# monahand1023/imageclust

Measured on AMD Instinct MI355X. Metric: images/sec (embed+Ward), higher is better.
Workload: dtype bf16; 1 GPU; the metric's size (configs[2]'s N=100000) on 1 GPU: 100000 synthetic 224x224x3 images (structured, seed 20250217; 100000 on this rank), ResNet50-v1 bf16 batch=256 -> 2048-d pooled E -> Ward min=5 max=50 (merge loop on GPU0) -> cluster ids on host; n_images_total=100000, embed_dim=2048, weights=synthetic seed 1, device=AMD Radeon Graphics (gfx950:sramecc+:xnack-)

## Files before the change

### imageclust_amd/_lib.py

```python
import ctypes as C
import os

import numpy as np

_HERE = os.path.dirname(os.path.abspath(__file__))
SO_PATH = os.environ.get("ICL_SO_PATH") or os.path.join(_HERE, "libimageclust_hip.so")

ICL_OK = 0
ICL_ERR_ARG, ICL_ERR_CONSTRAINT, ICL_ERR_HIP, ICL_ERR_NOMODEL, ICL_ERR_IO, ICL_ERR_UNSUPPORTED, ICL_ERR_OVERSIZE, ICL_ERR_NOMEM = range(1, 9)
HEAD_POOLED, HEAD_DENSE0 = 2048, 1000
PREC_FP32, PREC_BF16, PREC_BF16X3 = 0, 1, 2
UPDATE_EXACT, UPDATE_LW = 0, 1
SYNTH_NOISE, SYNTH_STRUCTURED = 0, 1
TILES_AUTO, TILES_LOCAL, TILES_DISTRIBUTED = 0, 1, 2
MERGE_GPU0, MERGE_SHARDED = 0, 1
CONV_P8_OFF, CONV_P8_AUTO, CONV_P8_ALL = 0, 1, 2
CONV_SPLIT = 16
ROWS_SINGLE, ROWS_EXACT_BATCH, ROWS_LW_BOUND, ROWS_LW_FAST, ROWS_SINGLE_APART = 0, 1, 2, 3, 4
FILE_FAIL_NEXT_LEADER = 0x100
MANY_MID_AUTO, MANY_MID_OFF, MANY_MID_ON = 0, 1, 2
PNG_HOST, PNG_GPU = 0, 1
ENTROPY_HOST, ENTROPY_GPU = 0, 1
K_CONV, K_DIST_EXACT, K_DIST_MFMA, K_ROWMIN, K_UPDATE, K_EMBED_OTHER, K_CONV64 = range(7)
K_NAMES = ["conv_igemm_kernel<*,128>", "ward_dist_exact_kernel", "dist_mfma_kernel", "row_argmin_*_kernel",
# ... 59 lines not shown
    ("icl_jpeg_encode_rgb", _int, [_vp, _i32, _i32, _i32, _vp, _i64, _pi64]),
    ("icl_jpeg_encode_rgb_dev", _int, [_vp, _vp, _vp, _vp, _vp, _i64, _i32, _vp, _i32, _i64, _vp]),
    ("icl_downsize_image_file", _int, [C.c_char_p, _i64, _i32, _vp, _i64, _pi64, _vp]),
    ("icl_downsize_image_mem", _int, [_vp, _i64, _i64, _i32, _vp, _i64, _pi64, _vp]),
    ("icl_downsize_images", _int, [_vp, _vp, _i64, _i64, _i32, _i32, _vp, _i64, _vp, _vp]),
    ("icl_downsize_images_mem", _int, [_vp, _vp, _vp, _i64, _i64, _i32, _i32, _vp, _i64, _vp, _vp]),
    ("icl_last_downsize_stats", _int, [_vp, _pi64, _pi64, _pi64, _pi64, _pi64, _pi64, _vp]),
    ("icl_set_batch", _int, [_vp, _int]),
    ("icl_set_conv_options", _int, [_vp, _int]),
    ("icl_conv_stats", _int, [_vp, _vp, _vp]),
    ("icl_set_forward_prune", _int, [_vp, _int]),
    ("icl_forward_prune_stats", _int, [_vp, _vp]),
    ("icl_set_forward_prune_fused", _int, [_vp, _int]),
    ("icl_forward_prune_fused_stats", _int, [_vp, _vp]),
    ("icl_set_stem_max_blocks", _int, [_vp, _int]),
    ("icl_bottleneck56_sub", _int, [_vp, _vp, _int, _int, _int] + [_vp] * 9 + [_int, _int, _vp]),
    ("icl_conv1x1_mapped", _int, [_vp, _vp, _int, _int, _int, _int, _vp, _int, _vp, _vp, _vp, _int, _vp]),
    ("icl_conv_split_launches", _int, [_vp, _vp]),
    ("icl_conv2d_fused", _int, [_vp, _int, _vp, _int, _int, _int, _vp, _int, _int, _int, _int, _vp, _vp, _vp, _int, _vp]),
    ("icl_conv2d_dual", _int, [_vp, _int, _vp, _int, _int, _int, _vp, _vp, _int, _int, _vp, _int, _int, _vp, _vp, _int, _vp]),
    ("icl_embed_taps", _int, [_vp, _int, _vp, _int, _int, _vp]),
    ("icl_stem_pool", _int, [_vp, _int, _vp, _int, _vp]),
    ("icl_bottleneck56", _int, [_vp, _vp, _int, _int, _int, _int] + [_vp] * 13),
    ("icl_calc_optimal_clusters", _int, [_i64, _i64, _i64, _pi64]),
    ("icl_ward_distance_matrix", _int, [_vp, _vp, _vp, _i64, _i32, _vp, _i64]),
    ("icl_ward_distance_matrix_dev", _int, [_vp, _vp, _vp, _i64, _i32, _vp, _i64]),
    ("icl_merge_centroid", _int, [_vp, _vp, _i64, _vp, _i64, _i32, _vp]),
    ("icl_update_distance_matrix", _int, [_vp, _vp, _i64, _i64, _vp, _vp, _i32, _i64, _i64, _vp, _i64]),
    ("icl_find_closest", _int, [_vp, _vp, _i64, _i64, _pi64, _pi64]),
    ("icl_find_closest_dev", _int, [_vp, _vp, _i64, _i64, _pi64, _pi64]),
    ("icl_group_create", _int, [_pi32, _i32, C.POINTER(_vp)]),
    ("icl_group_destroy", None, [_vp]),
# ... 494 lines not shown

    def set_conv_options(self, p8_mode=1):
        check(self.h, self.L.icl_set_conv_options(self.h, p8_mode))

    def set_forward_prune(self, on=True):
        check(self.h, self.L.icl_set_forward_prune(self.h, 1 if on else 0))

    def forward_prune_stats(self):
        a = C.c_int64(0)
        check(self.h, self.L.icl_forward_prune_stats(self.h, C.byref(a)))
        return a.value

    def set_forward_prune_fused(self, on=True):
        check(self.h, self.L.icl_set_forward_prune_fused(self.h, 1 if on else 0))

    def set_stem_max_blocks(self, max_blocks=0):
        check(self.h, self.L.icl_set_stem_max_blocks(self.h, int(max_blocks)))

    def forward_prune_fused_stats(self):
        a = C.c_int64(0)
        check(self.h, self.L.icl_forward_prune_fused_stats(self.h, C.byref(a)))
        return a.value

    def embed_u8(self, imgs, head=HEAD_POOLED, prec=PREC_FP32):
        imgs = np.ascontiguousarray(imgs, np.uint8).reshape(-1, IMG_BYTES)
        n = imgs.shape[0]
        out = np.empty((n, head), np.float32)
        check(self.h, self.L.icl_embed_u8(self.h, imgs.ctypes.data, n, head, prec, out.ctypes.data))
        return out

# ... 229 lines not shown
        Cout, _, k, _ = w.shape
        Ho = (H + 2 * pad - k) // stride + 1
        y = np.empty((B, Ho, Ho, Cout), np.float32)
        sc = np.ascontiguousarray(scale, np.float32)
        sh = np.ascontiguousarray(shift, np.float32)
        r = None if residual is None else np.ascontiguousarray(residual, np.float32)
        check(self.h, self.L.icl_conv2d_fused(self.h, prec, x.ctypes.data, B, H, Cin, w.ctypes.data, Cout, k, stride, pad,
                                              sc.ctypes.data, sh.ctypes.data, None if r is None else r.ctypes.data,
                                              1 if relu else 0, y.ctypes.data))
        return y

    def conv1x1_mapped(self, x_nhwc, w, scale, shift, y_full, sub, residual=None, relu=True):
        f = lambda a: np.ascontiguousarray(a, np.float32)
        x, w, sc, sh = f(x_nhwc), f(w), f(scale), f(shift)
        y = np.array(y_full, np.float32, order="C", copy=True)
        B, H, _, Cout = y.shape
        Ho = (H - 1) // int(sub) + 1
        Cin = x.shape[3]
        assert x.shape == (B, Ho, Ho, Cin) and w.shape == (Cout, Cin) and sc.shape == (Cout,) and sh.shape == (Cout,)
        r = None if residual is None else f(residual)
        assert r is None or r.shape == y.shape
        check(self.h, self.L.icl_conv1x1_mapped(self.h, x.ctypes.data, B, H, int(sub), Cin, w.ctypes.data, Cout, sc.ctypes.data, sh.ctypes.data,
                                                None if r is None else r.ctypes.data, 1 if relu else 0, y.ctypes.data))
        return y

    def conv2d_dual(self, x_nhwc, w1, x2_nhwc, w2, stride2, scale, shift, relu=True, prec=PREC_FP32):
        f = lambda a: np.ascontiguousarray(a, np.float32)
        x, x2, w1, w2, sc, sh = f(x_nhwc), f(x2_nhwc), f(w1), f(w2), f(scale), f(shift)
        B, Ho, _, Cin = x.shape
        _, H2, _, Cin2 = x2.shape
        Cout = w1.shape[0]
        assert x2.shape[0] == B and w1.shape == (Cout, Cin) and w2.shape == (Cout, Cin2) and sc.shape == (Cout,) and sh.shape == (Cout,)
        y = np.empty((B, Ho, Ho, Cout), np.float32)
        check(self.h, self.L.icl_conv2d_dual(self.h, prec, x.ctypes.data, B, Ho, Cin, w1.ctypes.data, x2.ctypes.data, H2, Cin2, w2.ctypes.data,
                                             int(stride2), Cout, sc.ctypes.data, sh.ctypes.data, 1 if relu else 0, y.ctypes.data))
        return y

# ... 783 lines not shown
```

### imageclust_amd/csrc/conv_p8.h

```cpp
#pragma once
#include "conv_select.h"
#include "mfma_tile.h"
#include "resnet_fused.h"

template <int MW, int NWV>
struct p8_geom {
    static_assert(MW * NWV == 8 && (NWV == 4 || NWV == 2), "8 waves");
    static constexpr int BM = MW * 128, BN = NWV * 64;
    static constexpr int PX = MW, PW = NWV / 2;
    static constexpr int SX = PX * 8192, SW = PW * 8192;
    static constexpr int O_WA = 0, O_XA = SW, O_WB = SW + SX, O_XB = 2 * SW + SX;
    static constexpr int BUF = 2 * (SW + SX);
    static constexpr int LDS = 2 * BUF;
    static constexpr int INFLIGHT = 2 * PW + PX;
    static_assert(INFLIGHT == 6 && LDS <= 160 * 1024, "counted vmcnt(6); the CU's 160 KiB");
};

template <int NP>
__device__ __forceinline__ void p8_dma(const i32x4_t &srd, const unsigned (&voff)[NP], unsigned soff, unsigned lds0)
{
    unsigned keep;
    if constexpr (NP == 1) {
        asm volatile("s_mov_b32 %0, m0\n\ts_mov_b32 m0, %4\n\ts_nop 4\n\tbuffer_load_dwordx4 %1, %2, %3 offen lds\n\ts_mov_b32 m0, %0"
                     : "=&s"(keep)
// ... 22 lines not shown
__global__ __launch_bounds__(512) void conv_p8_kernel(const conv_args p)
{
    static_assert(!(SPLIT && DUAL), "the split form covers single-operand layers");
    static_assert(!(SPLIT && X3), "the split form is bf16 only");
    typedef p8_geom<MW, NWV> G;
    typedef unsigned u32x2_t __attribute__((ext_vector_type(2)));
    constexpr int PX = G::PX, PW = G::PW;
    __shared__ __attribute__((aligned(1024))) unsigned char smem[G::LDS];
    const int tid = threadIdx.x, lane = tid & 63;
    const int wid = __builtin_amdgcn_readfirstlane(tid >> 6);
    const int wr = wid / NWV, wc = wid % NWV;
    const int grp = wid >> 2;
    const int ntile = p.gx * p.gy;
    const int role = SPLIT ? (int)blockIdx.x / ntile : 0;
    const int tile = xcd_remap((int)blockIdx.x - role * ntile, ntile);
    const int m0 = (tile / p.gy) * G::BM, n0 = (tile % p.gy) * G::BN;
    const i32x4_t xsrd = bn56_srd(p.X, (unsigned)((size_t)p.B * p.H * p.W * p.Cin * 2));
    const i32x4_t wsrd = bn56_srd(p.Wt, (unsigned)((size_t)p.Cout * p.K * 2));
    const i32x4_t x2srd = DUAL ? bn56_srd(p.X2, (unsigned)((size_t)p.B * p.H2 * p.W2 * p.Cin2 * 2)) : xsrd;

    unsigned vx[2][PX], vw[2][PW], vx2[DUAL ? 2 : 1][PX], vmask[PX];
#pragma unroll
    for (int j = 0; j < PW; ++j) {
        const int sr = (j * 8 + wid) * 8 + (lane >> 3);
        const unsigned ls16 = (unsigned)(((lane & 7) ^ ((sr >> 1) & 7)) << 4);
#pragma unroll
        for (int h = 0; h < 2; ++h) {
            const int wrow = n0 + (sr >> 5) * 64 + h * 32 + (sr & 31);
            vw[h][j] = (unsigned)wrow * (unsigned)p.K * 2u + ls16;
        }
    }
// ... 364 lines not shown
```

### imageclust_amd/csrc/conv_select.h

```cpp
#pragma once
#include <cstddef>
#include <cstdint>

#include "prune_map.h"

struct conv_args {
    const void *X;
    const void *Wt;
    void *Y;
    const void *R;
    const float *scale;
    const float *shift;
    const void *zero;
    int B, H, W, Cin, Ho, Wo, Cout, KH, KW, stride, pad, relu;
    int64_t M;
    int K;
    int gx, gy;
    const void *X2;
    int H2, W2, Cin2, stride2;
    void *sk_part;
    int *sk_flag;
    int sk_epoch;
    prune_map omap;
};

#define CONV_PREC_FP32 0
#define CONV_PREC_BF16 1
#define CONV_PREC_BF16X3 2
#define CONV_TILE_M 128
#define CONV_ROW_BYTES 128
#define HALO_MAXP 12
#ifndef P8_AUTO_MIN_NT
// ... 204 lines not shown
    *ngroups = g < 1 ? 1 : g;
}
static inline unsigned fwd_stem_blocks(int64_t units, int per_cu, int ncu, int max_blocks = 0)
{
    const int64_t g = units < (int64_t)per_cu * ncu ? units : (int64_t)per_cu * ncu;
    return (unsigned)(max_blocks > 0 && max_blocks < g ? max_blocks : g);
}

struct fwd_opts {
    conv_opts conv;
    int fuse;
    int prune;
    int stem_per_cu;
    int prune_fused = 1;
    int stem_max_blocks = 0;
};

enum fwd_kind { FWD_STEM2_POOL, FWD_STEM_POOL, FWD_STEM, FWD_MAXPOOL, FWD_BNECK56, FWD_CONV, FWD_AVGPOOL, FWD_FC };
enum { FWD_X = 0, FWD_T1 = 1, FWD_T2 = 2, FWD_DS = 3, FWD_Y = 4, FWD_NONE = -1 };

struct fwd_step {
    int kind;
    int layer;
    bool ds;
    bool pruned;
    int sub;
    conv_args a;
    conv_choice c;
    int x, y, r, x2;
    unsigned blocks, threads;
};
struct fwd_plan {
    std::vector<fwd_step> steps;
    int out = FWD_X;
    int H = 56, C = 64;
    int B = 0;
    int pruned = 0;
    const char *err = nullptr;
    int err_layer = 0;
};

static inline bool plan_pruned_block(const icl_conv_rec &r2, const icl_conv_rec &r3, int s, int B, const conv_opts &o, conv_args *p2, conv_args *p3)
{
    if (s <= 1) return false;
    const int prec = CONV_PREC_BF16;
    const conv_args u2 = conv_plain(nullptr, nullptr, nullptr, nullptr, nullptr, nullptr, nullptr, B, r2.hin, r2.cin, r2.cout, r2.k, r2.stride, r2.pad, 1);
    conv_args u3 = conv_plain(nullptr, nullptr, nullptr, nullptr, nullptr, nullptr, nullptr, B, r3.hin, r3.cin, r3.cout, 1, 1, 0, 1);
    *p2 = conv_plain(nullptr, nullptr, nullptr, nullptr, nullptr, nullptr, nullptr, B, r2.hin, r2.cin, r2.cout, r2.k, s, r2.pad, 1);
    *p3 = conv_plain(nullptr, nullptr, nullptr, nullptr, nullptr, nullptr, nullptr, B, p2->Ho, r3.cin, r3.cout, 1, 1, 0, 1);
    u3.R = p3->R = &u3;
    p3->omap = prune_map_make(s, r3.hout, r3.hout);
    if (u2.K != r2.cin * r2.k * r2.k || u3.K != r3.cin || p2->Ho != p3->omap.Ho) return false;
    const bool same = conv_same_arithmetic(conv_select(prec, u2, o), conv_select(prec, *p2, o)) && conv_same_arithmetic(conv_select(prec, u3, o), conv_select(prec, *p3, o));
    p3->R = nullptr;
    return same;
}

static inline fwd_plan forward_make_plan(const icl_conv_rec *recs, int nconv, int prec, int B, bool dense_head, int tap, const fwd_opts &o)
{
    fwd_plan p;
    p.B = B;
    const bool bf16 = prec == CONV_PREC_BF16, x3 = prec == CONV_PREC_BF16X3;
    const int bk = bf16 ? 64 : 32;
    int x = FWD_X, y = FWD_Y;
    auto add = [&](int kind, int layer, int xi, int yi) -> fwd_step & {
        fwd_step s = {};
        s.kind = kind; s.layer = layer; s.x = xi; s.y = yi; s.r = s.x2 = FWD_NONE;
        p.steps.push_back(s);
        return p.steps.back();
    };
// ... 67 lines not shown
            conv(ci + 1, FWD_T1, FWD_T2, FWD_NONE, c2.hin, c2.stride, nullptr, FWD_NONE);
            if (has_ds) {
                const icl_conv_rec &d = recs[ci + 3];
                if (d.cin % bk || c3.cout % 128) return fail("fused downsample shape not supported", ci + 2);
                conv(ci + 2, FWD_T2, y, FWD_NONE, c3.hin, 1, nullptr, x);
            } else {
                conv(ci + 2, FWD_T2, y, x, c3.hin, 1, nullptr, FWD_NONE);
            }
        }
        std::swap(x, y);
        ci = cn;
    }
    for (const fwd_step &s : p.steps)
        if (s.kind == FWD_CONV && s.c.family == CONV_UNSUPPORTED) return fail(s.c.why, s.layer);
    p.out = x;
    if (tap >= 0) return p;
    fwd_step &ap = add(FWD_AVGPOOL, 0, x, FWD_NONE);
    ap.blocks = (unsigned)conv_ceil_div((int64_t)B * 2048, 256);
    ap.threads = 256;
    if (dense_head) {
        fwd_step &fc = add(FWD_FC, 0, FWD_NONE, FWD_NONE);
        const int64_t want = conv_ceil_div((int64_t)B * 1000, 4);
        fc.blocks = (unsigned)(want < 4096 ? want : 4096);
        fc.threads = 256;
    }
    return p;
}
```

### imageclust_amd/csrc/conv_wr.h

```cpp
#pragma once
#include "conv_select.h"
#include "mfma_tile.h"
#include "prune_map.h"
#include "resnet_fused.h"

template <int NP>
__device__ __forceinline__ void wr_dma_chunk(const i32x4_t &srd, unsigned v0, unsigned v1, unsigned soff, unsigned lds0)
{
    unsigned keep;
    if constexpr (NP == 2)
        asm volatile("s_mov_b32 %0, m0\n\ts_mov_b32 m0, %5\n\ts_nop 4\n\tbuffer_load_dwordx4 %1, %3, %4 offen lds\n\t"
                     "s_mov_b32 m0, %6\n\ts_nop 0\n\tbuffer_load_dwordx4 %2, %3, %4 offen lds\n\ts_mov_b32 m0, %0"
                     : "=&s"(keep)
                     : "v"(v0), "v"(v1), "s"(srd), "s"(soff), "s"(lds0), "s"(lds0 + 4096u)
                     : "memory");
    else
        asm volatile("s_mov_b32 %0, m0\n\ts_mov_b32 m0, %4\n\ts_nop 4\n\tbuffer_load_dwordx4 %1, %2, %3 offen lds\n\ts_mov_b32 m0, %0"
                     : "=&s"(keep)
                     : "v"(v0), "s"(srd), "s"(soff), "s"(lds0)
                     : "memory");
}
template <int KC, int PT>
__device__ __forceinline__ void wr_dma(const i32x4_t &srd, unsigned v0, unsigned v1, unsigned lds0)
{
    static_assert(PT == 64 || PT == 32, "64- or 32-pixel tiles");
#pragma unroll
    for (int c = 0; c < KC; ++c) wr_dma_chunk<PT / 32>(srd, v0, v1, 128u * c, lds0 + (unsigned)(PT * 128) * c);
}

struct wr_args {
    const uint16_t *X;
    const uint16_t *W;
    const uint16_t *R;
    uint16_t *Y;
    const float *scale, *shift;
    int M, N, relu;
    int nslices, nworkers;
    prune_map pm;
};

template <int K, int NS, int MT, bool RES, bool MAP = false>
__global__ __launch_bounds__(256, (K == 256 && MT == 2) ? 3 : 2) void conv_wr_kernel(const wr_args p)
{
    typedef unsigned u32x2_t __attribute__((ext_vector_type(2)));
    typedef unsigned u32x4_t __attribute__((ext_vector_type(4)));
    constexpr int KC = K / 64, KF = K / 32;
    constexpr int CW = NS / 4, NT = CW / 16;
    constexpr int PT = 16 * MT;
    constexpr int ABYTES = KC * PT * 128;
    static_assert(NT % 2 == 0 && NT * KF * 4 <= 128 && (MT == 4 || MT == 2), "pairs of accumulator tiles for the lane swap; <= 128 VGPRs of weights");
    __shared__ __attribute__((aligned(1024))) unsigned char smem[2 * ABYTES];
    const int tid = threadIdx.x, lane = tid & 63;
    const int wid = __builtin_amdgcn_readfirstlane(tid >> 6);
    const int l15 = lane & 15, q = lane >> 4;
    const int xcd = (int)blockIdx.x & 7, rr = (int)blockIdx.x >> 3;
    const int slice = rr % p.nslices, worker = (rr / p.nslices) * 8 + xcd;
    const int n0 = slice * NS + wid * CW;
    const int ntiles = (p.M + PT - 1) / PT;
    if (worker >= ntiles) return;

    u32x4_t wreg[NT][KF];
#pragma unroll
    for (int nt = 0; nt < NT; ++nt)
#pragma unroll
        for (int kf = 0; kf < KF; ++kf) wreg[nt][kf] = *reinterpret_cast<const u32x4_t *>(p.W + (size_t)(n0 + 16 * nt + l15) * K + 32 * kf + 8 * q);
    asm volatile("s_waitcnt vmcnt(0)" ::: "memory");
#pragma unroll
    for (int nt = 0; nt < NT; ++nt)
#pragma unroll
        for (int kf = 0; kf < KF; ++kf) asm volatile("" : "+v"(wreg[nt][kf]));
    const int cbl = (q & 1) * 16 + (q >> 1) * 8;
    float sc[NT / 2][8], sh[NT / 2][8];
#pragma unroll
    for (int i = 0; i < NT / 2; ++i) {
// ... 4 lines not shown
        sh[i][0] = b0.x; sh[i][1] = b0.y; sh[i][2] = b0.z; sh[i][3] = b0.w; sh[i][4] = b1.x; sh[i][5] = b1.y; sh[i][6] = b1.z; sh[i][7] = b1.w;
    }
    const i32x4_t xsrd = bn56_srd(p.X, (unsigned)((size_t)p.M * K * 2));
    const unsigned lds0 = __builtin_amdgcn_readfirstlane(lds_addr_of(smem) + wid * 1024);
    int drow[2];
    unsigned dsw[2];
#pragma unroll
    for (int j = 0; j < 2; ++j) {
        drow[j] = (j * 4 + wid) * 8 + (lane >> 3);
        dsw[j] = (unsigned)(((lane & 7) ^ ((drow[j] >> 1) & 7)) << 4);
    }
    auto stage = [&](int tile, int buf) {
        unsigned v[2];
#pragma unroll
        for (int j = 0; j < 2; ++j) {
            const int m = tile * PT + drow[j];
            v[j] = (tile < ntiles && m < p.M) ? (unsigned)m * (unsigned)(K * 2) + dsw[j] : BN56_OOB;
        }
        wr_dma<KC, PT>(xsrd, v[0], v[1], lds0 + buf * ABYTES);
    };
    const int fsw = (l15 >> 1) & 7;
    unsigned xoff[2];
#pragma unroll
    for (int s = 0; s < 2; ++s) xoff[s] = (unsigned)(l15 * 128 + ((((4 * s + q) ^ fsw) & 7) << 4));

    typedef uint16_t elem;
    const size_t ypix = MAP ? (size_t)(p.M / (p.pm.Ho * p.pm.Wo)) * p.pm.H * p.pm.W : (size_t)p.M;
    const __amdgpu_buffer_rsrc_t rsrd = __builtin_amdgcn_make_buffer_rsrc((void *)(RES ? p.R : p.Y), 0, (int)(ypix * p.N * 2), 0x00020000);
    const __amdgpu_buffer_rsrc_t ysrd = __builtin_amdgcn_make_buffer_rsrc((void *)p.Y, 0, (int)(ypix * p.N * 2), 0x00020000);
    u32x4_t rv[MT][NT / 2];
    auto row_off = [&](int tile, int mt) -> unsigned {
        const int64_t m = (int64_t)tile * PT + mt * 16 + l15;
        if constexpr (MAP) {
            if (!(tile < ntiles && m < p.M)) return BN56_OOB;
            return (unsigned)((prune_map_pixel(p.pm, (unsigned)m) * p.N + n0 + cbl) * 2);
        }
        return (tile < ntiles && m < p.M) ? (unsigned)((m * p.N + n0 + cbl) * 2) : BN56_OOB;
    };
    auto load_res = [&](int tile) {
        if (!RES) return;
#pragma unroll
        for (int mt = 0; mt < MT; ++mt) {
            const unsigned o = row_off(tile, mt);
#pragma unroll
            for (int i = 0; i < NT / 2; ++i) rv[mt][i] = __builtin_amdgcn_raw_buffer_load_b128(rsrd, (int)o, i * 64, 0);
        }
    };
// ... 76 lines not shown
        }
        return;
    }
    if (res) hipLaunchKernelGGL((conv_wr_kernel<K, NS, MT, true>), grid, dim3(256), 0, strm, w);
    else hipLaunchKernelGGL((conv_wr_kernel<K, NS, MT, false>), grid, dim3(256), 0, strm, w);
}
static void launch_conv_wr(icl_ctx *ctx, const conv_args &a, const conv_choice &c)
{
    hipStream_t strm = ctx->cur_stream ? ctx->cur_stream : ctx->stream;
    wr_args w;
    w.X = (const uint16_t *)a.X; w.W = (const uint16_t *)a.Wt; w.R = (const uint16_t *)a.R; w.Y = (uint16_t *)a.Y;
    w.scale = a.scale; w.shift = a.shift; w.M = (int)a.M; w.N = a.Cout; w.relu = a.relu;
    w.pm = a.omap;
    w.nslices = c.slices;
    w.nworkers = c.workers;
    const dim3 grid(c.blocks);
    if (c.wr_k == 128) launch_conv_wr_t<128, 256, 4>(strm, w, grid, c.res);
    else if (c.wr_k == 256 && c.wr_mt == 4) launch_conv_wr_t<256, 128, 4>(strm, w, grid, c.res);
    else if (c.wr_k == 256) launch_conv_wr_t<256, 128, 2>(strm, w, grid, c.res);
    else launch_conv_wr_t<512, 128, 2>(strm, w, grid, c.res);
}
```

### imageclust_amd/csrc/icl_common.h

```cpp
#pragma once
#include <hip/hip_runtime.h>

#include <condition_variable>
#include <cstdarg>
#include <cstdint>
#include <cstdio>
#include <functional>
#include <mutex>
#include <string>
#include <vector>

#include "../../include/icl_model_format.h"
#include "../../include/imageclust.h"

#define ICL_MAXF 3.40282346638528859811704183484516925e+38f

struct icl_ctx;
int icl_fail(icl_ctx *ctx, int code, const char *fmt, ...);
static inline hipStream_t icl_main_stream(const icl_ctx *ctx);

#define ICL_HIP(ctx, call)                                                                                     \
    do {                                                                                                       \
        hipError_t e__ = (call);                                                                               \
        if (e__ != hipSuccess)                                                                                 \
// ... 135 lines not shown
    double requests_ms[3] = {0, 0, 0};
    icl_jenc_ws *jenc = nullptr;
    dz_totals downsize_last;
    icl_dev_grow nearest;
    int nearest_splits = 0;
    int64_t nearest_stats[4] = {0, 0, 0, 0};
    icl_dev_grow pairs;
    int64_t pairs_stats[4] = {0, 0, 0, 0};
    icl_dev_grow fit;
    int64_t fit_stats[4] = {0, 0, 0, 0};
    int64_t between_stats[5] = {0, 0, 0, 0, 0};
    std::vector<const void *> lds_optin;
    int fwd_prune_fused = 1;
    int64_t pruned_fused = 0;
    int stem_max_blocks = 0;
};

static inline hipStream_t icl_main_stream(const icl_ctx *ctx) { return ctx->stream; }

struct icl_device_guard {
    int prev = -1;
    bool ok = true;
    explicit icl_device_guard(int dev)
    {
        if (hipGetDevice(&prev) != hipSuccess) prev = -1;
        if (prev != dev) ok = (hipSetDevice(dev) == hipSuccess);
    }
    ~icl_device_guard()
    {
        if (prev >= 0) (void)hipSetDevice(prev);
// ... 116 lines not shown
```

### imageclust_amd/csrc/icl_core.hip

```cpp
#include "icl_common.h"

#include <cstring>

static thread_local std::string g_tls_err;

int icl_fail(icl_ctx *ctx, int code, const char *fmt, ...)
{
    char buf[1024];
    va_list ap;
    va_start(ap, fmt);
    vsnprintf(buf, sizeof buf, fmt, ap);
    va_end(ap);
    if (ctx) ctx->err = buf;
    g_tls_err = buf;
    return code;
}

extern "C" const char *icl_version(void) { return "imageclust_hip 0.1 (gfx950)"; }

extern "C" const char *icl_last_error(icl_ctx *ctx) { return ctx ? ctx->err.c_str() : g_tls_err.c_str(); }

extern "C" int icl_create(int device, icl_ctx **out)
{
    if (!out) return icl_fail(nullptr, ICL_ERR_ARG, "icl_create: out is NULL");
// ... 179 lines not shown
{
    if (!ctx || !pruned_blocks) return icl_fail(ctx, ICL_ERR_ARG, "icl_forward_prune_stats: NULL argument");
    std::lock_guard<std::mutex> lk(ctx->mu);
    *pruned_blocks = ctx->pruned_blocks;
    return ICL_OK;
}

extern "C" int icl_set_forward_prune_fused(icl_ctx *ctx, int on)
{
    if (!ctx || on < 0 || on > 1) return icl_fail(ctx, ICL_ERR_ARG, "icl_set_forward_prune_fused: on must be 0 or 1");
    std::lock_guard<std::mutex> lk(ctx->mu);
    ctx->fwd_prune_fused = on;
    return ICL_OK;
}

extern "C" int icl_set_stem_max_blocks(icl_ctx *ctx, int max_blocks)
{
    if (!ctx || max_blocks < 0) return icl_fail(ctx, ICL_ERR_ARG, "icl_set_stem_max_blocks: max_blocks must be 0 (no cap) or positive");
    std::lock_guard<std::mutex> lk(ctx->mu);
    ctx->stem_max_blocks = max_blocks;
    return ICL_OK;
}

extern "C" int icl_forward_prune_fused_stats(icl_ctx *ctx, int64_t *pruned_launches)
{
    if (!ctx || !pruned_launches) return icl_fail(ctx, ICL_ERR_ARG, "icl_forward_prune_fused_stats: NULL argument");
    std::lock_guard<std::mutex> lk(ctx->mu);
    *pruned_launches = ctx->pruned_fused;
    return ICL_OK;
}
// ... 138 lines not shown
```

### imageclust_amd/csrc/resnet.hip

```cpp
#include "icl_common.h"
#include "mfma_tile.h"
#include "resnet_model.h"

#include <algorithm>
#include <cmath>
#include <cstring>
#include <deque>
#include <new>
#include <thread>
#include <type_traits>
#include <vector>

#include "conv_select.h"
static_assert(CONV_PREC_FP32 == ICL_PREC_FP32 && CONV_PREC_BF16 == ICL_PREC_BF16 && CONV_PREC_BF16X3 == ICL_PREC_BF16X3 && CONV_TILE_M == CV_BM && CONV_ROW_BYTES == CV_ROWB,
              "conv_select.h restates these constants");

#include "resnet_fused.h"
#include "conv_p8.h"
#include "conv_wr.h"

template <typename T, int BN>
struct conv_resid {
    static constexpr int NPASS = 64 / (256 / (BN / T::KE));
    uint4 v[2][NPASS];
// ... 615 lines not shown
        }
#pragma unroll
        for (int off = 32; off > 0; off >>= 1) s += __shfl_down(s, off, 64);
        if (lane == 0) y[b * nout + o] = s + bias[o];
    }
}

template <typename T, int BN, bool DUAL, bool EARLY>
static void launch_conv_igemm(icl_ctx *ctx, const conv_args &a, const conv_choice &c)
{
    icl_lds_optin(ctx, (const void *)conv_igemm_kernel<T, BN, DUAL, 2, EARLY>, (int)conv_igemm_lds(BN, 2));
    hipLaunchKernelGGL((conv_igemm_kernel<T, BN, DUAL, 2, EARLY>), dim3(c.blocks), dim3(c.threads), c.lds, ctx->cur_stream ? ctx->cur_stream : ctx->stream, a);
}

struct fwd_env {
    int conv_mode, wr_pt256, fuse;
};
static const fwd_env &forward_env()
{
    static const fwd_env e = [] {
        const char *m = getenv("ICL_CONV_MODE"), *p = getenv("ICL_WR_PT256"), *f = getenv("ICL_FUSE");
        return fwd_env{m ? atoi(m) : 1, p && atoi(p) == 32 ? 32 : 64, f ? atoi(f) : 15};
    }();
    return e;
}
static int fuse_mask() { return forward_env().fuse; }
static conv_opts conv_opts_of(const icl_ctx *ctx)
{
    const fwd_env &e = forward_env();
    return conv_opts{ctx->conv_p8, ctx->conv_wr, ctx->conv_sk, ctx->conv_sk_min_k, e.conv_mode, e.wr_pt256, ctx->prop.multiProcessorCount};
}

template <typename T>
static int launch_conv_t(icl_ctx *ctx, int prec, const conv_args &real, const conv_choice &c)
{
    constexpr bool X3 = is_x3<T>::value;
    if (c.family == CONV_UNSUPPORTED) return icl_fail(ctx, ICL_ERR_UNSUPPORTED, "%s", c.why);
// ... 12 lines not shown
    case CONV_HALO:
        if (c.bn == 128) c.ring == 3 ? launch_conv3x3_halo<T, 128, 3>(ctx, a, c) : launch_conv3x3_halo<T, 128, 2>(ctx, a, c);
        else c.ring == 3 ? launch_conv3x3_halo<T, 64, 3>(ctx, a, c) : launch_conv3x3_halo<T, 64, 2>(ctx, a, c);
        break;
    default:
        if (c.dual) c.early ? launch_conv_igemm<T, 128, true, true>(ctx, a, c) : launch_conv_igemm<T, 128, true, false>(ctx, a, c);
        else if (c.bn == 128) c.early ? launch_conv_igemm<T, 128, false, true>(ctx, a, c) : launch_conv_igemm<T, 128, false, false>(ctx, a, c);
        else c.early ? launch_conv_igemm<T, 64, false, true>(ctx, a, c) : launch_conv_igemm<T, 64, false, false>(ctx, a, c);
    }
    ++ctx->conv_launches[c.counter];
    ctx->conv_sk_launches += split;
    ICL_HIP(ctx, hipGetLastError());
    return ICL_OK;
}

static int launch_conv_prec(icl_ctx *ctx, int prec, const conv_args &a)
{
    const conv_choice c = conv_select(prec, a, conv_opts_of(ctx));
    return with_prec(prec, [&](auto t) { return launch_conv_t<decltype(t)>(ctx, prec, a, c); });
}

static inline conv_args conv_stem(const icl_model *m, const void *Wt, void *Y, int B, int gx)
{
    const conv_layer &L = m->conv[0];
    conv_args a = conv_plain(nullptr, Wt, Y, nullptr, L.scale, L.shift, m->zero, B, 224, 3, 64, 7, 2, 3, 1);
    a.K = STEM_K;
    a.gx = gx;
    a.gy = 1;
    return a;
}

static int from_dev(icl_ctx *ctx, int prec, const void *src, size_t n, float *dst)
// ... 75 lines not shown
        dev_guard &dx = io.buf(), &dx2 = io.buf(), &dw = io.buf(), &dy = io.buf(), &dz = io.buf(), &dsc = io.buf(), &dsh = io.buf();
        ICL_TRY(upload_as(ctx, prec, &dx.p, x, nx));
        ICL_TRY(upload_as(ctx, prec, &dx2.p, x2, nx2));
        ICL_TRY(zero_page(ctx, "icl_conv2d_dual", dz));
        ICL_TRY(upload_as(ctx, prec, &dw.p, wp.data(), wp.size()));
        ICL_TRY(upload_as(ctx, ICL_PREC_FP32, &dsc.p, scale, (size_t)Cout));
        ICL_TRY(upload_as(ctx, ICL_PREC_FP32, &dsh.p, shift, (size_t)Cout));
        ICL_TRY(icl_dev_alloc(ctx, dy, ny * prec_act_bytes(prec), "icl_conv2d_dual: output"));
        conv_args a = conv_plain(dx.p, dw.p, dy.p, nullptr, (const float *)dsc.p, (const float *)dsh.p, dz.p, B, Ho, Cin, Cout, 1, 1, 0, relu);
        conv_add_operand(a, dx2.p, H2, Cin2, stride2);
        io.returns(prec, dy.p, ny);
        return launch_conv_prec(ctx, prec, a);
    });
}

extern "C" int icl_conv1x1_mapped(icl_ctx *ctx, const float *x, int B, int H, int sub, int Cin, const float *w, int Cout, const float *scale,
                                  const float *shift, const float *residual, int relu, float *y)
{
    if (!ctx || !x || !w || !scale || !shift || !y || B < 1 || H < 1 || sub < 1 || Cin < 1 || Cout < 1)
        return icl_fail(ctx, ICL_ERR_ARG, "icl_conv1x1_mapped: bad argument");
    if ((int64_t)B * H * H * Cout * 2 >= (1LL << 31)) return icl_fail(ctx, ICL_ERR_UNSUPPORTED, "icl_conv1x1_mapped: the full tensor exceeds the kernel's 32-bit buffer offsets");
    return run_entry(ctx, "icl_conv1x1_mapped", false, y, [&](entry_io &io) -> int {
        const int prec = ICL_PREC_BF16;
        const prune_map pm = prune_map_make(sub, H, H);
        const size_t nx = (size_t)B * pm.Ho * pm.Wo * Cin, ny = (size_t)B * H * H * Cout;
        dev_guard &dx = io.buf(), &dw = io.buf(), &dr = io.buf(), &dy = io.buf(), &dz = io.buf(), &dsc = io.buf(), &dsh = io.buf();
        ICL_TRY(upload_as(ctx, prec, &dx.p, x, nx));
        ICL_TRY(zero_page(ctx, "icl_conv1x1_mapped", dz));
        ICL_TRY(upload_as(ctx, prec, &dw.p, w, (size_t)Cout * Cin));
        if (residual) ICL_TRY(upload_as(ctx, prec, &dr.p, residual, ny));
        ICL_TRY(upload_as(ctx, prec, &dy.p, y, ny));
        ICL_TRY(upload_as(ctx, ICL_PREC_FP32, &dsc.p, scale, (size_t)Cout));
        ICL_TRY(upload_as(ctx, ICL_PREC_FP32, &dsh.p, shift, (size_t)Cout));
        conv_args a = conv_plain(dx.p, dw.p, dy.p, dr.p, (const float *)dsc.p, (const float *)dsh.p, dz.p, B, pm.Ho, Cin, Cout, 1, 1, 0, relu);
        a.omap = pm;
        io.returns(prec, dy.p, ny);
        if (conv_select(prec, a, conv_opts_of(ctx)).family != CONV_WR) return icl_fail(ctx, ICL_ERR_UNSUPPORTED, "icl_conv1x1_mapped: Cin = %d, Cout = %d is no shape of the streaming kernel's mapped form", Cin, Cout);
        return launch_conv_prec(ctx, prec, a);
    });
}

static int stem_per_cu(int prec, int fuse)
{
    const size_t cu_lds = (size_t)160 * 1024;
    if (prec == ICL_PREC_BF16 && (fuse & 1) && (fuse & 8)) return std::max<int>(1, std::min<int>(5, (int)(cu_lds / stem2_lds_bytes())));
    if (prec == ICL_PREC_BF16X3 || (fuse & 1)) return std::max<int>(1, (int)(cu_lds / (prec == ICL_PREC_BF16 ? stem_pool_lds_bytes<BF16>() : stem_pool_lds_bytes<F32>())));
    return std::max<int>(1, (int)(cu_lds / (prec == ICL_PREC_BF16 ? stem_lds_bytes<BF16>() : stem_lds_bytes<F32>())));
}
static fwd_opts forward_opts_of(const icl_ctx *ctx, int prec)
{
    return fwd_opts{conv_opts_of(ctx), fuse_mask(), ctx->fwd_prune, stem_per_cu(prec, fuse_mask()), ctx->fwd_prune_fused, ctx->stem_max_blocks};
}

template <typename T>
static void launch_stem_pool(icl_ctx *ctx, int prec, const uint8_t *d_img, int B, void *pooled, unsigned grid, hipStream_t strm)
{
    icl_model *m = ctx->model;
    if (prec == ICL_PREC_BF16 && (fuse_mask() & 8)) {
        const conv_layer &L0 = m->conv[0];
        icl_prof_scope ps(ctx, ICL_K_CONV64, 2.0 * (double)B * 112 * 112 * 64 * 147, 0.0);
        const int nunits = B * SP_STRIPS;
        hipLaunchKernelGGL(stem2_pool_kernel, dim3(grid), dim3(256), stem2_lds_bytes(), strm, d_img, (const uint16_t *)L0.wfold, L0.shift, (uint16_t *)pooled, nunits);
        return;
    }
    constexpr bool SPLIT = is_x3<T>::value;
    typedef typename std::conditional<SPLIT, F32, T>::type TS;
// ... 97 lines not shown
            }
            break;
        case FWD_MAXPOOL:
            if constexpr (!is_x3<T>::value) {
                icl_prof_scope ps(ctx, ICL_K_EMBED_OTHER, 0.0, (double)B * (802816.0 + 200704.0) * sizeof(elem));
                hipLaunchKernelGGL((maxpool_kernel<T>), dim3(s.blocks), dim3(s.threads), 0, strm, (const elem *)buf[s.x], B, 112, 64, (elem *)buf[s.y]);
            }
            break;
        case FWD_BNECK56:
            ICL_TRY(launch_bneck56(ctx, L, m->conv[s.layer + 1], m->conv[s.layer + 2], s.ds ? &m->conv[s.layer + 3] : nullptr, buf[s.x], buf[s.y], B, s.sub, strm));
            ctx->pruned_fused += s.sub == 2;
            break;
        case FWD_CONV: {
            conv_args a = s.a;
            a.X = buf[s.x]; a.Y = buf[s.y]; a.R = s.r != FWD_NONE ? buf[s.r] : nullptr; a.zero = m->zero;
            if (s.ds) {
                a.Wt = L.wfused[prec]; a.scale = m->ones; a.shift = L.shift_fused; a.X2 = buf[s.x2];
            } else {
                a.Wt = L.w[prec]; a.scale = L.scale; a.shift = L.shift;
            }
            ICL_TRY(launch_conv_t<T>(ctx, prec, a, s.c));
            ctx->pruned_blocks += s.pruned;
            break;
        }
        case FWD_AVGPOOL: {
            icl_prof_scope ps(ctx, ICL_K_EMBED_OTHER, 0.0, (double)B * 49.0 * 2048.0 * (is_x3<T>::value ? 4 : sizeof(elem)));
            hipLaunchKernelGGL((avgpool_kernel<T>), dim3(s.blocks), dim3(s.threads), 0, strm, (const elem *)buf[s.x], B, 49, ICL_FEAT_DIM, pooled, (int64_t)ICL_FEAT_DIM);
            break;
        }
        default: {
// ... 242 lines not shown
```

### include/imageclust.h

```cpp
#ifndef IMAGECLUST_H
#define IMAGECLUST_H
#include <stdint.h>

#ifdef __cplusplus
extern "C" {
#endif

typedef struct icl_ctx icl_ctx;

enum {
    ICL_OK = 0,
    ICL_ERR_ARG = 1,
    ICL_ERR_CONSTRAINT = 2,
    ICL_ERR_HIP = 3,
    ICL_ERR_NOMODEL = 4,
    ICL_ERR_IO = 5,
    ICL_ERR_UNSUPPORTED = 6,
    ICL_ERR_OVERSIZE = 7,
    ICL_ERR_NOMEM = 8
};

enum { ICL_HEAD_POOLED = 2048,
       ICL_HEAD_DENSE0 = 1000   };
enum { ICL_PREC_FP32 = 0,
// ... 49 lines not shown
int icl_jpeg_coefs_file_host(const char *path, int sub_bits, int16_t *coefs, int64_t cap, int64_t *need, int32_t *info );
enum { ICL_PNG_HOST = 0, ICL_PNG_GPU = 1 };
int icl_set_png_options(icl_ctx *ctx, int png_mode);
int icl_last_png_stats(icl_ctx *ctx, int64_t *gpu_pngs, int64_t *host_pngs, int64_t *redone_on_host, int64_t *stream_bytes);
int icl_png_raw_files(icl_ctx *ctx, const char *const *paths, int64_t n, int stage, uint8_t *raw, int64_t cap, int64_t *offsets ,
                      int32_t *state );
int icl_png_raw_file_host(const char *path, int stage, uint8_t *raw, int64_t cap, int64_t *need, int32_t *info );
int icl_png_raw_mem_host(const uint8_t *data, int64_t bytes, int stage, uint8_t *raw, int64_t cap, int64_t *need, int32_t *info );
int icl_set_batch(icl_ctx *ctx, int batch);
enum { ICL_CONV_P8_OFF = 0, ICL_CONV_P8_AUTO = 1, ICL_CONV_P8_ALL = 2, ICL_CONV_SPLIT = 16 };
int icl_set_conv_options(icl_ctx *ctx, int p8_mode);
int icl_set_forward_prune(icl_ctx *ctx, int on);
int icl_forward_prune_stats(icl_ctx *ctx, int64_t *pruned_blocks);
int icl_set_forward_prune_fused(icl_ctx *ctx, int on);
int icl_forward_prune_fused_stats(icl_ctx *ctx, int64_t *pruned_launches);
int icl_set_stem_max_blocks(icl_ctx *ctx, int max_blocks);
int icl_conv_split_launches(icl_ctx *ctx, int64_t *launches);
int icl_conv_stats(icl_ctx *ctx, int64_t *p8_launches, int64_t *other_launches);
int icl_conv2d_fused(icl_ctx *ctx, int prec, const float *x, int B, int H, int Cin, const float *w, int Cout, int k,
                     int stride, int pad, const float *scale, const float *shift, const float *residual, int relu,
                     float *y);

int icl_conv2d_dual(icl_ctx *ctx, int prec, const float *x, int B, int Ho, int Cin, const float *w1, const float *x2, int H2, int Cin2,
                    const float *w2, int stride2, int Cout, const float *scale, const float *shift, int relu, float *y);
int icl_conv1x1_mapped(icl_ctx *ctx, const float *x, int B, int H, int sub, int Cin, const float *w, int Cout, const float *scale,
                       const float *shift, const float *residual, int relu, float *y);
int icl_embed_taps(icl_ctx *ctx, int prec, const uint8_t *hwc_rgb, int B, int tap, float *out);

int icl_stem_pool(icl_ctx *ctx, int prec, const uint8_t *hwc_rgb, int B, float *out);
int icl_bottleneck56(icl_ctx *ctx, const float *x, int B, int H, int W, int Cin, const float *w1, const float *sc1, const float *sh1,
// ... 217 lines not shown
```

Before: 76220 images/sec.

## Reverse tile walk order of convs that consume a freshly written activation

```diff
diff --git a/imageclust_amd/_lib.py b/imageclust_amd/_lib.py
--- a/imageclust_amd/_lib.py
+++ b/imageclust_amd/_lib.py
@@ -97,8 +97,11 @@
     ("icl_set_forward_prune_fused", _int, [_vp, _int]),
     ("icl_forward_prune_fused_stats", _int, [_vp, _vp]),
     ("icl_set_stem_max_blocks", _int, [_vp, _int]),
+    ("icl_set_forward_walk", _int, [_vp, _int]),
+    ("icl_set_entry_walk", _int, [_vp, _int, _int]),
     ("icl_bottleneck56_sub", _int, [_vp, _vp, _int, _int, _int] + [_vp] * 9 + [_int, _int, _vp]),
     ("icl_conv1x1_mapped", _int, [_vp, _vp, _int, _int, _int, _int, _vp, _int, _vp, _vp, _vp, _int, _vp]),
+    ("icl_conv1x1_mapped_hw", _int, [_vp, _vp, _int, _int, _int, _int, _int, _vp, _int, _vp, _vp, _vp, _int, _vp]),
     ("icl_conv_split_launches", _int, [_vp, _vp]),
     ("icl_conv2d_fused", _int, [_vp, _int, _vp, _int, _int, _int, _vp, _int, _int, _int, _int, _vp, _vp, _vp, _int, _vp]),
     ("icl_conv2d_dual", _int, [_vp, _int, _vp, _int, _int, _int, _vp, _vp, _int, _int, _vp, _int, _int, _vp, _vp, _int, _vp]),
@@ -623,6 +626,12 @@
     def set_forward_prune_fused(self, on=True):
         check(self.h, self.L.icl_set_forward_prune_fused(self.h, 1 if on else 0))
 
+    def set_forward_walk(self, mask):
+        check(self.h, self.L.icl_set_forward_walk(self.h, int(mask)))
+
+    def set_entry_walk(self, rev=0, fill=-1):
+        check(self.h, self.L.icl_set_entry_walk(self.h, int(rev), int(fill)))
+
     def set_stem_max_blocks(self, max_blocks=0):
         check(self.h, self.L.icl_set_stem_max_blocks(self.h, int(max_blocks)))
 
@@ -882,13 +891,13 @@
         f = lambda a: np.ascontiguousarray(a, np.float32)
         x, w, sc, sh = f(x_nhwc), f(w), f(scale), f(shift)
         y = np.array(y_full, np.float32, order="C", copy=True)
-        B, H, _, Cout = y.shape
-        Ho = (H - 1) // int(sub) + 1
+        B, H, Wd, Cout = y.shape
+        Ho, Wo = (H - 1) // int(sub) + 1, (Wd - 1) // int(sub) + 1
         Cin = x.shape[3]
-        assert x.shape == (B, Ho, Ho, Cin) and w.shape == (Cout, Cin) and sc.shape == (Cout,) and sh.shape == (Cout,)
+        assert x.shape == (B, Ho, Wo, Cin) and w.shape == (Cout, Cin) and sc.shape == (Cout,) and sh.shape == (Cout,)
         r = None if residual is None else f(residual)
         assert r is None or r.shape == y.shape
-        check(self.h, self.L.icl_conv1x1_mapped(self.h, x.ctypes.data, B, H, int(sub), Cin, w.ctypes.data, Cout, sc.ctypes.data, sh.ctypes.data,
+        check(self.h, self.L.icl_conv1x1_mapped_hw(self.h, x.ctypes.data, B, H, Wd, int(sub), Cin, w.ctypes.data, Cout, sc.ctypes.data, sh.ctypes.data,
                                                 None if r is None else r.ctypes.data, 1 if relu else 0, y.ctypes.data))
         return y
 
diff --git a/imageclust_amd/csrc/conv_p8.h b/imageclust_amd/csrc/conv_p8.h
--- a/imageclust_amd/csrc/conv_p8.h
+++ b/imageclust_amd/csrc/conv_p8.h
@@ -60,7 +60,7 @@
     const int ntile = p.gx * p.gy;
     const int role = SPLIT ? (int)blockIdx.x / ntile : 0;
     const int tile = xcd_remap((int)blockIdx.x - role * ntile, ntile);
-    const int m0 = (tile / p.gy) * G::BM, n0 = (tile % p.gy) * G::BN;
+    const int m0 = (p.rev ? p.gx - 1 - tile / p.gy : tile / p.gy) * G::BM, n0 = (tile % p.gy) * G::BN;
     const i32x4_t xsrd = bn56_srd(p.X, (unsigned)((size_t)p.B * p.H * p.W * p.Cin * 2));
     const i32x4_t wsrd = bn56_srd(p.Wt, (unsigned)((size_t)p.Cout * p.K * 2));
     const i32x4_t x2srd = DUAL ? bn56_srd(p.X2, (unsigned)((size_t)p.B * p.H2 * p.W2 * p.Cin2 * 2)) : xsrd;
diff --git a/imageclust_amd/csrc/conv_select.h b/imageclust_amd/csrc/conv_select.h
--- a/imageclust_amd/csrc/conv_select.h
+++ b/imageclust_amd/csrc/conv_select.h
@@ -16,6 +16,7 @@
     int64_t M;
     int K;
     int gx, gy;
+    int rev;
     const void *X2;
     int H2, W2, Cin2, stride2;
     void *sk_part;
@@ -250,6 +251,7 @@
     int stem_per_cu;
     int prune_fused = 1;
     int stem_max_blocks = 0;
+    int walk = 0;
 };
 
 enum fwd_kind { FWD_STEM2_POOL, FWD_STEM_POOL, FWD_STEM, FWD_MAXPOOL, FWD_BNECK56, FWD_CONV, FWD_AVGPOOL, FWD_FC };
@@ -265,6 +267,7 @@
     conv_choice c;
     int x, y, r, x2;
     unsigned blocks, threads;
+    bool rev;
 };
 struct fwd_plan {
     std::vector<fwd_step> steps;
@@ -290,6 +293,40 @@
     const bool same = conv_same_arithmetic(conv_select(prec, u2, o), conv_select(prec, *p2, o)) && conv_same_arithmetic(conv_select(prec, u3, o), conv_select(prec, *p3, o));
     p3->R = nullptr;
     return same;
+}
+
+#define FWD_WALK_C1 1
+#define FWD_WALK_C2 2
+#define FWD_WALK_C3 4
+#define FWD_WALK_BNECK56 8
+#ifndef FWD_WALK_DEFAULT
+#define FWD_WALK_DEFAULT FWD_WALK_C3
+#endif
+static inline bool conv_has_direction(const conv_choice &c) { return c.family == CONV_WR || c.family == CONV_P8; }
+static inline bool conv_one_round(const conv_choice &c, int ncu) { return (int64_t)c.gx * c.gy <= ncu; }
+static inline void plan_walk_directions(std::vector<fwd_step> &steps, const icl_conv_rec *recs, int walk, int ncu)
+{
+    enum { NO_ORDER = 0, ASCENDING = 1, DESCENDING = 2 };
+    int last[5] = {NO_ORDER, NO_ORDER, NO_ORDER, NO_ORDER, NO_ORDER};
+    for (fwd_step &s : steps) {
+        s.rev = false;
+        int dir = ASCENDING;
+        if (s.kind == FWD_CONV) {
+            if (conv_one_round(s.c, ncu)) {
+                dir = NO_ORDER;
+            } else if (conv_has_direction(s.c)) {
+                const int role = recs[s.layer].role;
+                const int bit = role == 1 ? FWD_WALK_C1 : role == 2 ? FWD_WALK_C2 : FWD_WALK_C3;
+                const int dom = role == 3 ? (s.r != FWD_NONE ? s.r : s.x2) : s.x;
+                if ((walk & bit) && dom != FWD_NONE && last[dom] == ASCENDING) {
+                    s.rev = true;
+                    dir = DESCENDING;
+                }
+            }
+        }
+        for (int b : {s.x, s.y, s.r, s.x2})
+            if (b != FWD_NONE) last[b] = dir;
+    }
 }
 
 static inline fwd_plan forward_make_plan(const icl_conv_rec *recs, int nconv, int prec, int B, bool dense_head, int tap, const fwd_opts &o)
@@ -387,6 +424,7 @@
     for (const fwd_step &s : p.steps)
         if (s.kind == FWD_CONV && s.c.family == CONV_UNSUPPORTED) return fail(s.c.why, s.layer);
     p.out = x;
+    if (bf16) plan_walk_directions(p.steps, recs, o.walk, o.conv.ncu);
     if (tap >= 0) return p;
     fwd_step &ap = add(FWD_AVGPOOL, 0, x, FWD_NONE);
     ap.blocks = (unsigned)conv_ceil_div((int64_t)B * 2048, 256);
diff --git a/imageclust_amd/csrc/conv_wr.h b/imageclust_amd/csrc/conv_wr.h
--- a/imageclust_amd/csrc/conv_wr.h
+++ b/imageclust_amd/csrc/conv_wr.h
@@ -36,6 +36,7 @@
     const float *scale, *shift;
     int M, N, relu;
     int nslices, nworkers;
+    int rev;
     prune_map pm;
 };
 
@@ -58,6 +59,7 @@
     const int n0 = slice * NS + wid * CW;
     const int ntiles = (p.M + PT - 1) / PT;
     if (worker >= ntiles) return;
+    const int tbase = p.rev ? ntiles - 1 : 0, tstep = p.rev ? -1 : 1;
 
     u32x4_t wreg[NT][KF];
 #pragma unroll
@@ -92,7 +94,7 @@
         unsigned v[2];
 #pragma unroll
         for (int j = 0; j < 2; ++j) {
-            const int m = tile * PT + drow[j];
+            const int m = (tbase + tstep * tile) * PT + drow[j];
             v[j] = (tile < ntiles && m < p.M) ? (unsigned)m * (unsigned)(K * 2) + dsw[j] : BN56_OOB;
         }
         wr_dma<KC, PT>(xsrd, v[0], v[1], lds0 + buf * ABYTES);
@@ -108,7 +110,7 @@
     const __amdgpu_buffer_rsrc_t ysrd = __builtin_amdgcn_make_buffer_rsrc((void *)p.Y, 0, (int)(ypix * p.N * 2), 0x00020000);
     u32x4_t rv[MT][NT / 2];
     auto row_off = [&](int tile, int mt) -> unsigned {
-        const int64_t m = (int64_t)tile * PT + mt * 16 + l15;
+        const int64_t m = (int64_t)(tbase + tstep * tile) * PT + mt * 16 + l15;
         if constexpr (MAP) {
             if (!(tile < ntiles && m < p.M)) return BN56_OOB;
             return (unsigned)((prune_map_pixel(p.pm, (unsigned)m) * p.N + n0 + cbl) * 2);
@@ -215,6 +217,7 @@
     w.pm = a.omap;
     w.nslices = c.slices;
     w.nworkers = c.workers;
+    w.rev = a.rev;
     const dim3 grid(c.blocks);
     if (c.wr_k == 128) launch_conv_wr_t<128, 256, 4>(strm, w, grid, c.res);
     else if (c.wr_k == 256 && c.wr_mt == 4) launch_conv_wr_t<256, 128, 4>(strm, w, grid, c.res);
diff --git a/imageclust_amd/csrc/icl_common.h b/imageclust_amd/csrc/icl_common.h
--- a/imageclust_amd/csrc/icl_common.h
+++ b/imageclust_amd/csrc/icl_common.h
@@ -173,6 +173,9 @@
     int fwd_prune_fused = 1;
     int64_t pruned_fused = 0;
     int stem_max_blocks = 0;
+    int fwd_walk = -1;
+    int entry_rev = 0;
+    int entry_fill = -1;
 };
 
 static inline hipStream_t icl_main_stream(const icl_ctx *ctx) { return ctx->stream; }
diff --git a/imageclust_amd/csrc/icl_core.hip b/imageclust_amd/csrc/icl_core.hip
--- a/imageclust_amd/csrc/icl_core.hip
+++ b/imageclust_amd/csrc/icl_core.hip
@@ -217,6 +217,23 @@
     return ICL_OK;
 }
 
+extern "C" int icl_set_forward_walk(icl_ctx *ctx, int mask)
+{
+    if (!ctx || mask < -1 || mask > 15) return icl_fail(ctx, ICL_ERR_ARG, "icl_set_forward_walk: mask must be 0 .. 15, or -1 for the default");
+    std::lock_guard<std::mutex> lk(ctx->mu);
+    ctx->fwd_walk = mask;
+    return ICL_OK;
+}
+
+extern "C" int icl_set_entry_walk(icl_ctx *ctx, int rev, int fill)
+{
+    if (!ctx || rev < 0 || rev > 1 || fill < -1 || fill > 0xffff) return icl_fail(ctx, ICL_ERR_ARG, "icl_set_entry_walk: rev must be 0 or 1, fill -1 or a 16-bit pattern");
+    std::lock_guard<std::mutex> lk(ctx->mu);
+    ctx->entry_rev = rev;
+    ctx->entry_fill = fill;
+    return ICL_OK;
+}
+
 extern "C" int icl_set_stem_max_blocks(icl_ctx *ctx, int max_blocks)
 {
     if (!ctx || max_blocks < 0) return icl_fail(ctx, ICL_ERR_ARG, "icl_set_stem_max_blocks: max_blocks must be 0 (no cap) or positive");
diff --git a/imageclust_amd/csrc/resnet.hip b/imageclust_amd/csrc/resnet.hip
--- a/imageclust_amd/csrc/resnet.hip
+++ b/imageclust_amd/csrc/resnet.hip
@@ -653,13 +653,13 @@
 }
 
 struct fwd_env {
-    int conv_mode, wr_pt256, fuse;
+    int conv_mode, wr_pt256, fuse, walk;
 };
 static const fwd_env &forward_env()
 {
     static const fwd_env e = [] {
-        const char *m = getenv("ICL_CONV_MODE"), *p = getenv("ICL_WR_PT256"), *f = getenv("ICL_FUSE");
-        return fwd_env{m ? atoi(m) : 1, p && atoi(p) == 32 ? 32 : 64, f ? atoi(f) : 15};
+        const char *m = getenv("ICL_CONV_MODE"), *p = getenv("ICL_WR_PT256"), *f = getenv("ICL_FUSE"), *w = getenv("ICL_WALK");
+        return fwd_env{m ? atoi(m) : 1, p && atoi(p) == 32 ? 32 : 64, f ? atoi(f) : 15, w ? atoi(w) & 15 : FWD_WALK_DEFAULT};
     }();
     return e;
 }
@@ -702,8 +702,12 @@
     return ICL_OK;
 }
 
-static int launch_conv_prec(icl_ctx *ctx, int prec, const conv_args &a)
-{
+static int launch_conv_prec(icl_ctx *ctx, int prec, const conv_args &a0)
+{
+    conv_args a = a0;
+    a.rev = ctx->entry_rev;
+    if (ctx->entry_fill >= 0 && prec == ICL_PREC_BF16 && !a.omap.sub)
+        ICL_HIP(ctx, hipMemsetD16Async((hipDeviceptr_t)a.Y, (unsigned short)ctx->entry_fill, (size_t)a.M * a.Cout, ctx->stream));
     const conv_choice c = conv_select(prec, a, conv_opts_of(ctx));
     return with_prec(prec, [&](auto t) { return launch_conv_t<decltype(t)>(ctx, prec, a, c); });
 }
@@ -809,16 +813,16 @@
     });
 }
 
-extern "C" int icl_conv1x1_mapped(icl_ctx *ctx, const float *x, int B, int H, int sub, int Cin, const float *w, int Cout, const float *scale,
-                                  const float *shift, const float *residual, int relu, float *y)
-{
-    if (!ctx || !x || !w || !scale || !shift || !y || B < 1 || H < 1 || sub < 1 || Cin < 1 || Cout < 1)
+extern "C" int icl_conv1x1_mapped_hw(icl_ctx *ctx, const float *x, int B, int H, int W, int sub, int Cin, const float *w, int Cout, const float *scale,
+                                     const float *shift, const float *residual, int relu, float *y)
+{
+    if (!ctx || !x || !w || !scale || !shift || !y || B < 1 || H < 1 || W < 1 || sub < 1 || Cin < 1 || Cout < 1)
         return icl_fail(ctx, ICL_ERR_ARG, "icl_conv1x1_mapped: bad argument");
-    if ((int64_t)B * H * H * Cout * 2 >= (1LL << 31)) return icl_fail(ctx, ICL_ERR_UNSUPPORTED, "icl_conv1x1_mapped: the full tensor exceeds the kernel's 32-bit buffer offsets");
+    if ((int64_t)B * H * W * Cout * 2 >= (1LL << 31)) return icl_fail(ctx, ICL_ERR_UNSUPPORTED, "icl_conv1x1_mapped: the full tensor exceeds the kernel's 32-bit buffer offsets");
     return run_entry(ctx, "icl_conv1x1_mapped", false, y, [&](entry_io &io) -> int {
         const int prec = ICL_PREC_BF16;
-        const prune_map pm = prune_map_make(sub, H, H);
-        const size_t nx = (size_t)B * pm.Ho * pm.Wo * Cin, ny = (size_t)B * H * H * Cout;
+        const prune_map pm = prune_map_make(sub, H, W);
+        const size_t nx = (size_t)B * pm.Ho * pm.Wo * Cin, ny = (size_t)B * H * W * Cout;
         dev_guard &dx = io.buf(), &dw = io.buf(), &dr = io.buf(), &dy = io.buf(), &dz = io.buf(), &dsc = io.buf(), &dsh = io.buf();
         ICL_TRY(upload_as(ctx, prec, &dx.p, x, nx));
         ICL_TRY(zero_page(ctx, "icl_conv1x1_mapped", dz));
@@ -828,12 +832,19 @@
         ICL_TRY(upload_as(ctx, ICL_PREC_FP32, &dsc.p, scale, (size_t)Cout));
         ICL_TRY(upload_as(ctx, ICL_PREC_FP32, &dsh.p, shift, (size_t)Cout));
         conv_args a = conv_plain(dx.p, dw.p, dy.p, dr.p, (const float *)dsc.p, (const float *)dsh.p, dz.p, B, pm.Ho, Cin, Cout, 1, 1, 0, relu);
+        a.W = a.Wo = pm.Wo;
+        a.M = (int64_t)B * pm.Ho * pm.Wo;
         a.omap = pm;
         io.returns(prec, dy.p, ny);
         if (conv_select(prec, a, conv_opts_of(ctx)).family != CONV_WR) return icl_fail(ctx, ICL_ERR_UNSUPPORTED, "icl_conv1x1_mapped: Cin = %d, Cout = %d is no shape of the streaming kernel's mapped form", Cin, Cout);
         return launch_conv_prec(ctx, prec, a);
     });
 }
+extern "C" int icl_conv1x1_mapped(icl_ctx *ctx, const float *x, int B, int H, int sub, int Cin, const float *w, int Cout, const float *scale,
+                                  const float *shift, const float *residual, int relu, float *y)
+{
+    return icl_conv1x1_mapped_hw(ctx, x, B, H, H, sub, Cin, w, Cout, scale, shift, residual, relu, y);
+}
 
 static int stem_per_cu(int prec, int fuse)
 {
@@ -844,7 +855,8 @@
 }
 static fwd_opts forward_opts_of(const icl_ctx *ctx, int prec)
 {
-    return fwd_opts{conv_opts_of(ctx), fuse_mask(), ctx->fwd_prune, stem_per_cu(prec, fuse_mask()), ctx->fwd_prune_fused, ctx->stem_max_blocks};
+    return fwd_opts{conv_opts_of(ctx), fuse_mask(), ctx->fwd_prune, stem_per_cu(prec, fuse_mask()), ctx->fwd_prune_fused, ctx->stem_max_blocks,
+                    ctx->fwd_walk >= 0 ? ctx->fwd_walk : forward_env().walk};
 }
 
 template <typename T>
@@ -972,6 +984,7 @@
         case FWD_CONV: {
             conv_args a = s.a;
             a.X = buf[s.x]; a.Y = buf[s.y]; a.R = s.r != FWD_NONE ? buf[s.r] : nullptr; a.zero = m->zero;
+            a.rev = s.rev;
             if (s.ds) {
                 a.Wt = L.wfused[prec]; a.scale = m->ones; a.shift = L.shift_fused; a.X2 = buf[s.x2];
             } else {
diff --git a/include/imageclust.h b/include/imageclust.h
--- a/include/imageclust.h
+++ b/include/imageclust.h
@@ -87,6 +87,10 @@
 int icl_forward_prune_stats(icl_ctx *ctx, int64_t *pruned_blocks);
 int icl_set_forward_prune_fused(icl_ctx *ctx, int on);
 int icl_forward_prune_fused_stats(icl_ctx *ctx, int64_t *pruned_launches);
+int icl_conv1x1_mapped_hw(icl_ctx *ctx, const float *x, int B, int H, int W, int sub, int Cin, const float *w, int Cout, const float *scale,
+                          const float *shift, const float *residual, int relu, float *y);
+int icl_set_forward_walk(icl_ctx *ctx, int mask);
+int icl_set_entry_walk(icl_ctx *ctx, int rev, int fill);
 int icl_set_stem_max_blocks(icl_ctx *ctx, int max_blocks);
 int icl_conv_split_launches(icl_ctx *ctx, int64_t *launches);
 int icl_conv_stats(icl_ctx *ctx, int64_t *p8_launches, int64_t *other_launches);
diff --git a/scratch/resource_usage.py b/scratch/resource_usage.py
--- /dev/null
+++ b/scratch/resource_usage.py
@@ -0,0 +1,38 @@
+#!/usr/bin/env python3
+import re
+import sys
+
+KEYS = ["VGPRs", "AGPRs", "TotalSGPRs", "ScratchSize [bytes/lane]", "Occupancy [waves/SIMD]", "SGPRs Spill", "VGPRs Spill", "LDS Size [bytes/block]"]
+
+
+def usage(path):
+    out, cur = {}, None
+    for ln in open(path):
+        m = re.search(r"remark: Function Name: (\S+)", ln)
+        if m:
+            cur = out.setdefault(m.group(1), {})
+            continue
+        m = re.search(r"remark:\s+([A-Za-z][^:]*): (\d+) \[-Rpass", ln)
+        if m and cur is not None:
+            cur[m.group(1)] = int(m.group(2))
+    return out
+
+
+def main():
+    pat, a, b = sys.argv[1], usage(sys.argv[2]), usage(sys.argv[3])
+    bad = 0
+    print("%-64s %s" % ("kernel: parent -> branch", " | ".join(k.split(" [")[0] for k in KEYS)))
+    for k in sorted(b):
+        if not re.search(pat, k):
+            continue
+        p, q = a.get(k, {}), b[k]
+        cells = ["%s -> %s" % (p.get(key, "-"), q.get(key, "-")) if p.get(key) != q.get(key) else "%s" % q.get(key, "-") for key in KEYS]
+        worse = any(q.get(key, 0) > p.get(key, 0) for key in ("ScratchSize [bytes/lane]", "SGPRs Spill", "VGPRs Spill")) or q.get(KEYS[4], 0) < p.get(KEYS[4], 0)
+        bad += worse
+        print("%-64s %s%s" % (k, " | ".join(cells), "   <-- WORSE" if worse else ""))
+    print("no new spill, scratch or loss of occupancy" if not bad else "%d kernels worse" % bad)
+    return 1 if bad else 0
+
+
+if __name__ == "__main__":
+    sys.exit(main())
```

Result: no change. 76190 images/sec, median of 2 (-0.0%).
